# sloisel/MultiGridBarrier.jl

Measured on AMD Instinct MI355X. Metric: Newton iters/sec + wall-clock to converge, 2D P2 p-Laplace L=9, higher is better.
Workload: dtype f64

## Files before the change

multigridbarrier.jl_amd/csrc/driver.cpp:

```cpp
#include <chrono>
#include <cstdio>
#include <cstdlib>
#include <cmath>
#include <cstring>
#include <functional>
#include <limits>

#include "problem.hpp"

using namespace mgbhip;

namespace {

constexpr double EPS = std::numeric_limits<double>::epsilon();

bool debug_on() {
    static const bool on = env_on("MGBHIP_DEBUG");
    return on;
}
#define DBG(...) do { if (debug_on()) { fprintf(stderr, __VA_ARGS__); } } while (0)

struct Stop {
    double lambda_tol;
    double theta;
    int (*fn)(double, double, double, double, double, double, void*) = nullptr;
    void* user = nullptr;
    bool operator()(double ymin, double ynext, double gmin, double gnorm_next, double ndecmin, double ndec) const {
        if (fn) return fn(ymin, ynext, gmin, gnorm_next, ndecmin, ndec, user) != 0;
        const bool exact = (ynext >= ymin) && (gnorm_next >= theta * gmin);
        if (lambda_tol >= 0) return (ndec < lambda_tol) || exact;
        return exact;
    }
};

struct NewtonResult {
    int k = 0;
    bool converged = false;
    double y = 0;
};

struct VecStats { double sumsq, bad; };

VecStats vec_stats(mgbhip_problem* P, int level, const double* d_v, int64_t len) {
    hipStream_t st = P->stream();
    launch_vec_stats(d_v, len, P->d_scratch.p, P->d_scal.p + 2, st, P->own_mask(level));
    P->read_scalars(2, 2);
    if (P->sharded()) P->allreduce_host(P->pin.d + 2, 2, 0);
    return VecStats{P->pin.d[2], P->pin.d[3]};
}

double dev_dot(mgbhip_problem* P, int level, const double* a, const double* b, int64_t len) {
    hipStream_t st = P->stream();
    launch_dot(a, b, len, P->d_scratch.p, P->d_scal.p + 4, st, P->own_mask(level));
    P->read_scalars(4, 1);
    if (P->sharded()) P->allreduce_host(P->pin.d + 4, 1, 0);
    return P->pin.d[4];
}

struct NewtonCtx {
    mgbhip_problem* P;
    int level;
    const double* d_zJ;
    const double* d_c;
    int64_t m;
    double F0(const double* d_s) { return P->eval_f0(level, d_s, d_zJ, d_c); }
    void F1(const double* d_s, double* d_out, double* d_part) { P->eval_f1(level, d_s, d_zJ, d_c, d_out, P->sharded() ? d_part : nullptr); }
    const double* rhs_of_g() const { return P->sharded() ? P->d_gpart.p : P->d_g.p; }
    void F2(const double* d_s) { P->eval_f2(level, d_s, d_zJ, d_c, false, rhs_of_g()); }
};

bool trial_values(NewtonCtx& C, double& ynext, double& gnorm_next, int32_t* moved = nullptr, const double* step = nullptr,
                  bool* restrict_fused_out = nullptr) {
    mgbhip_problem* P = C.P;
    hipStream_t st = P->stream();
    const bool onfly = step && P->can_fuse_step(C.level);
    if (step) {
        ++P->step_stamp;
        if (!onfly) launch_step(P->d_x.p, P->d_nv.p, *step, P->d_xn.p, C.m, P->d_flag.p, P->step_stamp, st);
        P->touch();
    }
    const bool fused = !P->dense;
    static const bool fuse_restrict = !env_on("MGBHIP_NO_FUSED_RESTRICT");
    TrialRestrict fuse;
    TrialPoint point{};
    if (onfly) {
        point = TrialPoint{P->d_x.p, P->d_nv.p, *step};
        fuse = TrialRestrict{P->d_x.p, P->d_nv.p, *step, P->d_xn.p, P->d_flag.p, P->step_stamp};
    }
    const bool restrict_fused = P->eval_f01_launch(C.level, P->d_xn.p, C.d_zJ, C.d_c, P->d_gn.p, P->sharded() ? P->d_gnpart.p : nullptr, fused,
                                                   onfly ? &point : nullptr, (fused && fuse_restrict) ? &fuse : nullptr);
    if (restrict_fused_out) *restrict_fused_out = restrict_fused;
    if (onfly && !restrict_fused) launch_step(P->d_x.p, P->d_nv.p, *step, P->d_xn.p, C.m, P->d_flag.p, P->step_stamp, st);
    const double seq = P->next_seq();
    launch_trial_finish(P->d_gn.p, C.m, P->d_scratch.p, fused ? P->d_partials.p : nullptr, elem_grid(P->p, P->N), P->d_scal.p,
                        P->d_flag.p, P->pin.dev, st, P->own_mask(C.level), seq, restrict_fused);
    P->wait_results(seq);
    P->pin.i[0] = P->pin.d[4] == (double)P->step_stamp ? 1 : 0;
    if (P->sharded()) {
        P->pin.d[1] = (double)P->pin.i[0];
        P->allreduce_host(P->pin.d, 4, 0);
        P->pin.i[0] = P->pin.d[1] != 0.0 ? 1 : 0;
    }
    if (moved) *moved = P->pin.i[0];
    ynext = P->pin.d[0];
    if (!std::isfinite(ynext)) return false;
    if (P->pin.d[3] != 0.0 || !std::isfinite(P->pin.d[2])) return false;
    gnorm_next = std::sqrt(P->pin.d[2]);
    return true;
}

bool linesearch_backtracking(NewtonCtx& C, const mgbhip_options& opt, double y, double inc, double& ynext,
                             double& gnorm_next) {
    mgbhip_problem* P = C.P;
    hipStream_t st = P->stream();
    double s = 1.0;
    bool have = false;
    while (s > 0.0) {
        double yn, gn;
        int32_t moved = 0;
        if (trial_values(C, yn, gn, &moved, &s)) {
            have = true;
            ynext = yn;
            gnorm_next = gn;
            const bool stalled = (moved == 0);
            if (stalled || yn <= y - opt.ls_c1 * inc * s) return true;
        }
        s *= opt.ls_beta;
    }
    return have;
}

bool linesearch_illinois(NewtonCtx& C, const mgbhip_options& opt, double inc, double& ynext, double& gnorm_next) {
    mgbhip_problem* P = C.P;
    hipStream_t st = P->stream();
    struct Reject {};
    auto phi = [&](double sigma) -> double {
        launch_step(P->d_x.p, P->d_nv.p, sigma, P->d_xn.p, C.m, P->d_flag.p, ++P->step_stamp, st);
        P->touch();
        const double f = C.F0(P->d_xn.p);
        if (!std::isfinite(f)) throw Reject();
        C.F1(P->d_xn.p, P->d_gn.p, P->d_gnpart.p);
        const double v = dev_dot(P, C.level, P->d_gn.p, P->d_nv.p, C.m);
        if (!std::isfinite(v)) throw Reject();
        return v;
    };
    double s = 1.0;
    bool have = false;
    while (s > 0.0) {
        try {
            double a = 0.0, b = s, fa = inc, fb = phi(s), root = b;
            bool done = false;
            if (fa == 0) { root = a; done = true; }
            else if (fa * fb >= 0) { root = b; done = true; }
            for (int it = 0; it < 10000 && !done; ++it) {
                const double c = (a * fb - b * fa) / (fb - fa);
                const double fc = phi(c);
                if (c <= std::fmin(a, b) || c >= std::fmax(a, b) || fc * fa == 0 || fc * fb == 0) { root = c; done = true; break; }
                if (fb * fc < 0) { a = b; fa = fb; } else { fa /= 2; }
                b = c; fb = fc;
            }
            if (!done) throw Reject();
            launch_step(P->d_x.p, P->d_nv.p, root, P->d_xn.p, C.m, P->d_flag.p, ++P->step_stamp, st);
        P->touch();
            double yn, gn;
            if (!trial_values(C, yn, gn)) throw Reject();
            ynext = yn;
            gnorm_next = gn;
            return true;
        } catch (Reject&) {
        }
        s *= opt.ls_beta;
    }
    return have;
}

NewtonResult newton(NewtonCtx& C, const mgbhip_options& opt, const Stop& stop, int maxit) {
    mgbhip_problem* P = C.P;
    hipStream_t st = P->stream();
    NewtonResult R;
    P->d_x.zero(st, (size_t)C.m);
    P->touch();
    double y = C.F0(P->d_x.p);
    if (!std::isfinite(y)) throw InvalidArgument("newton: initial objective value is not finite");
    double ymin = y;
    if (P->sharded()) { P->d_gpart.ensure((size_t)C.m); P->d_gnpart.ensure((size_t)C.m); }
    C.F1(P->d_x.p, P->d_g.p, P->d_gpart.p);
    VecStats gs = vec_stats(P, C.level, P->d_g.p, C.m);
    if (gs.bad != 0.0 || !std::isfinite(gs.sumsq)) throw InvalidArgument("newton: initial gradient has non-finite entries");
    double gnorm = std::sqrt(gs.sumsq);
    double gmin = gnorm;
    double incmin = INFINITY;
    int k = 0;
    bool converged = false;
    Level& L = P->levels[C.level];
    struct RobustReset {
        MfSolver& s;
        ~RobustReset() { s.robust = false; }
    } robust_reset{L.solver};
    while (k < maxit && !converged) {
        ++k;
        C.F2(P->d_x.p);
        auto t0 = std::chrono::steady_clock::now();
        int fstatus = MGBHIP_OK;
        int leaf_flag = 0;
        for (int attempt = 0; attempt < 2; ++attempt) {
            P->factor(C.level, C.rhs_of_g());
            P->trisolve_carried(C.level, P->d_nv.p);
            const double seq = P->next_seq();
            launch_dir_finish(P->d_nv.p, P->d_g.p, C.m, P->d_scratch.p, P->d_scal.p, L.solver.status_flags_rw(), P->pin.dev, st,
                              P->own_mask(C.level), seq);
            L.solver.flags_cleared();
            P->wait_results(seq);
            P->pin.i[1] = P->pin.d[5] != 0.0 ? 1 : 0;
            leaf_flag |= P->pin.d[6] != 0.0 ? 1 : 0;
            P->pin.i[2] = leaf_flag;
            fstatus = MfSolver::status_from(P->pin.i + 1, L.solver.factored_condensed);
            if (P->sharded()) {
                P->pin.d[5] = fstatus != MGBHIP_OK ? 1.0 : 0.0;
                P->allreduce_host(P->pin.d + 2, 4, 0);
                fstatus = P->pin.d[5] != 0.0 ? MGBHIP_ERR_NOT_SPD : MGBHIP_OK;
            }
            const bool at_floor = std::fabs(P->pin.d[4]) <= EPS * std::fmax(std::fabs(y), 1.0);
            const bool suspicious = fstatus != MGBHIP_OK || P->pin.d[3] != 0.0 || !std::isfinite(P->pin.d[2]) ||
                                    (!(P->pin.d[4] > 0) && !at_floor);
            if (!suspicious || attempt == 1 || !L.solver.has_inverse_path() || L.solver.robust) break;
            DBG("newton[lev %d] k=%d: direction rejected (status %d, lambda^2=%.3e): refactoring with the substitution kernels\n",
                C.level, k, fstatus, P->pin.d[4]);
            L.solver.robust = true;
            L.H.drop_factors();
        }
        if (fstatus != MGBHIP_OK && P->lu_fallback(C.level, P->d_g.p, P->d_nv.p)) {
            DBG("newton[lev %d] k=%d: LDL' met a zero pivot; direction from the pivoted LU fallback\n", C.level, k);
            launch_dir_finish(P->d_nv.p, P->d_g.p, C.m, P->d_scratch.p, P->d_scal.p, L.solver.status_flags_rw(), P->pin.dev, st,
                              P->own_mask(C.level));
            L.solver.flags_cleared();
            MGB_HIP_CHECK(hipStreamSynchronize(st));
            fstatus = MGBHIP_OK;
        }
        P->cnt.solve_seconds += std::chrono::duration<double>(std::chrono::steady_clock::now() - t0).count();
        if (fstatus != MGBHIP_OK) {
            DBG("newton[lev %d] k=%d: Cholesky met a non-positive pivot (y=%.17g |g|=%.6e)\n", C.level, k, y, gnorm);
            converged = false;
            break;
        }
        if (P->pin.d[3] != 0.0 || !std::isfinite(P->pin.d[2])) throw InvalidArgument("newton: Newton direction has non-finite entries");
        const double inc = P->pin.d[4];
        DBG("newton[lev %d] k=%d y=%.17g |g|=%.6e lambda^2=%.6e\n", C.level, k, y, gnorm, inc);
        if (inc <= 0) {
            converged = std::fabs(inc) <= EPS * std::fmax(std::fabs(y), 1.0);
            break;
        }
        double ynext = y, gnorm_next = gnorm;
        bool moved = (opt.line_search == 1) ? linesearch_illinois(C, opt, inc, ynext, gnorm_next)
                                            : linesearch_backtracking(C, opt, y, inc, ynext, gnorm_next);
        if (!moved) {
            ynext = y;
            gnorm_next = gnorm;
        }
        if (stop(ymin, ynext, gmin, gnorm_next, std::sqrt(incmin), std::sqrt(inc))) converged = true;
        if (moved) {
            std::swap(P->d_x, P->d_xn);
            std::swap(P->d_g, P->d_gn);
            std::swap(P->d_gpart, P->d_gnpart);
        }
        y = ynext;
        gnorm = gnorm_next;
        gmin = std::fmin(gmin, gnorm);
        ymin = std::fmin(ymin, y);
        incmin = std::fmin(inc, incmin);
    }
    DBG("newton[lev %d] done k=%d converged=%d y=%.17g\n", C.level, k, (int)converged, y);
    R.k = k;
    R.converged = converged;
    R.y = y;
    P->cnt.newton += k;
    return R;
}

struct StepResult {
    bool converged;
    std::vector<int64_t> its;
};

StepResult mgb_step(mgbhip_problem* P, const double* d_c, const mgbhip_options& opt, bool finalize_now,
                    bool initial_step) {
    const int L = (int)P->levels.size();
    StepResult out;
    out.its.assign(L, 0);
    hipStream_t st = P->stream();
    const Stop sc{opt.stop_lambda_tol, opt.stop_theta, opt.stopping_criterion, opt.user};
    const Stop fin{-1.0, opt.finalize_theta};
    const size_t zn = (size_t)P->nu * P->n;
    auto eta = [&](int j, int J, const Stop& stop, int maxit) -> bool {
        (void)j;
        const int lev = J - 1;
        MGB_HIP_CHECK(hipMemcpyAsync(P->d_z0.p, P->d_z.p, zn * sizeof(double), hipMemcpyDeviceToDevice, st));
        NewtonCtx C{P, lev, P->d_z0.p, d_c, P->levels[lev].m};
        NewtonResult r = newton(C, opt, stop, maxit);
        out.its[lev] += r.k;
        if (r.converged) {
            const Level& Lv = P->levels[lev];
            StageScope scp(P->ctx->timers, "prolong");
            launch_csr_matvec(Lv.rows, Lv.Rptr.p, Lv.Rcol.p, Lv.Rval.p, P->d_x.p, P->d_z.p, true, false, st);
        }
        return r.converged;
    };
    std::function<bool(int, int)> dac = [&](int j, int J) -> bool {
        const int mn = (initial_step && J - j == 1) ? opt.maxit : opt.max_newton;
        if (eta(j, J, sc, mn)) return true;
        const int jmid = (j + J) / 2;
        if (jmid == j || jmid == J) return false;
        return dac(j, jmid) && dac(jmid, J);
    };
    bool converged = dac(0, L);
    if (finalize_now) {
        const bool foo = eta(L - 1, L, fin, opt.maxit);
        converged = converged && foo;
    }
    out.converged = converged;
    return out;
}

double c_dot_Dz(mgbhip_problem* P, const double* d_c) {
    hipStream_t st = P->stream();
    ElemParams E = P->elem_params(d_c);
    E.z0 = P->d_z.p;
    E.invn = 0.0;
    E.bw = nullptr;
    launch_elem(E, MODE_F0, st);
    launch_reduce_partials(P->d_partials.p, elem_grid(P->p, P->N), P->d_scal.p, st);
    double v;
    P->d_scal.download(&v, 1, st);
    MGB_HIP_CHECK(hipStreamSynchronize(st));
    if (P->sharded()) P->allreduce_host(&v, 1, 0);
    return v;
}

bool slack_feasible(mgbhip_problem* P, std::vector<double>& hbuf) {
    hipStream_t st = P->stream();
    hbuf.resize((size_t)P->n);
    MGB_HIP_CHECK(hipMemcpyAsync(hbuf.data(), P->d_z.p + (size_t)(P->nu - 1) * P->n, (size_t)P->n * sizeof(double),
                                 hipMemcpyDeviceToHost, st));
    MGB_HIP_CHECK(hipStreamSynchronize(st));
    double mx = -INFINITY;
    for (double v : hbuf) mx = std::fmax(mx, v);
    if (P->sharded()) P->allreduce_host(&mx, 1, 1);
    return mx < 0;
}

}

void trial_values_run(mgbhip_problem* P, int level, double step, double* y, int32_t* moved, int32_t* finite, int32_t* path) {
    NewtonCtx C{P, level, P->d_z0.p, P->d_c.p, P->levels[level].m};
    double yn = 0.0, gn = 0.0;
    const bool onfly = P->can_fuse_step(level);
    bool restrict_fused = false;
    *finite = trial_values(C, yn, gn, moved, &step, &restrict_fused) ? 1 : 0;
    *y = yn;
    *path = (onfly ? 1 : 0) | (restrict_fused ? 2 : 0);
}

int core_run(mgbhip_problem* P, double* z, const double* c, const mgbhip_options* optp, mgbhip_core_result* res) {
    const mgbhip_options opt = *optp;
    hipStream_t st = P->stream();
    const size_t zn = (size_t)P->nu * P->n;
    const size_t cn = (size_t)P->n * P->nD;
    const int L = (int)P->levels.size();
    P->prepare_all();
    P->d_z.upload(z, zn, st);
    P->d_c0.upload(c, cn, st);
    P->cnt = Counters();
    auto tb = std::chrono::steady_clock::now();
    auto now = [&] { return std::chrono::duration<double>(std::chrono::steady_clock::now() - tb).count(); };
    double t = opt.t;
    const double target = 1.0 / opt.tol;
    double kappa = opt.kappa;
    const double kappa0 = kappa;
    int k = 1;
    std::vector<double> hbuf;
    double t_first = INFINITY;
    std::vector<double> zhost;
    auto early = [&](double tt) -> bool {
        if (opt.early_stop_fn) {
            zhost.resize(zn);
            P->d_z.download(zhost.data(), zn, st);
            MGB_HIP_CHECK(hipStreamSynchronize(st));
            if (opt.early_stop_fn(zhost.data(), tt, opt.user) != 0) return true;
        }
        if (opt.early_stop != 1) return false;
        if (!slack_feasible(P, hbuf)) return false;
        t_first = std::fmin(t_first, tt);
        return tt >= 2 * t_first;
    };
    auto record = [&](int kk, const std::vector<int64_t>& its, bool add) {
        if (kk - 1 < res->cap_steps && res->its) {
            for (int l = 0; l < L; ++l) {
                if (add) res->its[(size_t)(kk - 1) * L + l] += its[l];
                else res->its[(size_t)(kk - 1) * L + l] = its[l];
            }
        }
    };
    auto setc = [&](double tt) { launch_scale_copy(P->d_c0.p, tt, P->d_c.p, (int64_t)cn, st); };
    res->failure_code = 0;
    res->L = L;
    if (res->times && res->cap_steps > 0) res->times[0] = now();
    setc(t);
    StepResult S = mgb_step(P, P->d_c.p, opt, opt.finalize && t >= target, true);
    if (!S.converged) {
        res->failure_code = 1;
        res->k = 1;
        res->t_final = t;
        res->t_elapsed = now();
        return MGBHIP_ERR_CONVERGENCE;
    }
    record(1, S.its, false);
    auto diag = [&](int kk) {
        if (kk - 1 < res->cap_steps) {
            if (res->ts) res->ts[kk - 1] = t;
            if (res->kappas) res->kappas[kk - 1] = kappa;
            if (res->c_dot_Dz) res->c_dot_Dz[kk - 1] = c_dot_Dz(P, P->d_c0.p);
        }
    };
    diag(1);
    bool stopped_early = false;
    while (t < target && kappa > 1 && k < opt.maxit) {
        if (early(t)) { stopped_early = true; break; }
        ++k;
        if (k - 1 < res->cap_steps && res->its)
            for (int l = 0; l < L; ++l) res->its[(size_t)(k - 1) * L + l] = 0;
        if (res->times && k - 1 < res->cap_steps) res->times[k - 1] = now();
        while (kappa > 1) {
            const double t1 = kappa * t;
            setc(t1);
            P->d_tmp.ensure(zn);
            MGB_HIP_CHECK(hipMemcpyAsync(P->d_tmp.p, P->d_z.p, zn * sizeof(double), hipMemcpyDeviceToDevice, st));
            S = mgb_step(P, P->d_c.p, opt, opt.finalize && t1 >= target, false);
            record(k, S.its, true);
            if (S.converged) {
                int64_t mx = 0;
                for (int64_t v : S.its) mx = std::max(mx, v);
                if ((double)mx <= opt.max_newton * 0.5) kappa = std::fmin(kappa0, kappa * kappa);
                t = t1;
                break;
            }
            MGB_HIP_CHECK(hipMemcpyAsync(P->d_z.p, P->d_tmp.p, zn * sizeof(double), hipMemcpyDeviceToDevice, st));
            kappa = std::sqrt(kappa);
        }
        diag(k);
    }
    bool converged = (t >= target) || stopped_early || early(t);
    res->k = k;
    res->t_final = t;
    res->t_elapsed = now();
    res->solve_seconds = P->cnt.solve_seconds;
    res->newton_iterations = P->cnt.newton;
    res->f0_evals = P->cnt.f0;
    res->f1_evals = P->cnt.f1;
    res->f2_evals = P->cnt.f2;
    res->factorizations = P->cnt.factor;
    P->d_z.download(z, zn, st);
    MGB_HIP_CHECK(hipStreamSynchronize(st));
    if (!converged) {
        res->failure_code = (kappa <= 1) ? 1 : 2;
        return MGBHIP_ERR_CONVERGENCE;
    }
    return MGBHIP_OK;
}

int matched_t_run(mgbhip_problem* P, const double* z, const double* c, double t_default, double* t_out) {
    hipStream_t st = P->stream();
    const size_t zn = (size_t)P->nu * P->n;
    const size_t cn = (size_t)P->n * P->nD;
    const int lev = (int)P->levels.size() - 1;
    const int64_t m = P->levels[lev].m;
    P->d_z0.upload(z, zn, st);
    P->d_c0.upload(c, cn, st);
    P->d_c.zero(st, cn);
    P->d_x.zero(st, (size_t)m);
    P->touch();
    *t_out = t_default;
    const bool sh = P->sharded();
    if (sh) { P->d_gpart.ensure((size_t)m); P->d_gnpart.ensure((size_t)m); }
    P->eval_f1(lev, P->d_x.p, P->d_z0.p, P->d_c.p, P->d_g.p, sh ? P->d_gpart.p : nullptr);
    P->eval_f1(lev, P->d_x.p, P->d_z0.p, P->d_c0.p, P->d_gn.p, sh ? P->d_gnpart.p : nullptr);
    launch_axpy(-1.0, P->d_g.p, P->d_gn.p, m, st);
    if (sh) launch_axpy(-1.0, P->d_gpart.p, P->d_gnpart.p, m, st);
    P->eval_f2(lev, P->d_x.p, P->d_z0.p, P->d_c0.p);
    if (sh) {
        P->d_tmp.ensure((size_t)m + 1);
        P->factor(lev, P->d_gpart.p);
        P->trisolve_carried(lev, P->d_tmp.p);
        int bad = P->levels[lev].solver.status(st) != MGBHIP_OK;
        MGB_HIP_CHECK(hipMemcpyAsync(P->d_nv.p, P->d_tmp.p, sizeof(double) * (size_t)m, hipMemcpyDeviceToDevice, st));
        P->levels[lev].H.drop_factors();
        P->factor(lev, P->d_gnpart.p);
        P->trisolve_carried(lev, P->d_tmp.p);
        bad |= P->levels[lev].solver.status(st) != MGBHIP_OK;
        MGB_HIP_CHECK(hipMemcpyAsync(P->d_xn.p, P->d_tmp.p, sizeof(double) * (size_t)m, hipMemcpyDeviceToDevice, st));
        double fb = bad ? 1.0 : 0.0;
        P->allreduce_host(&fb, 1, 0);
        if (fb != 0.0) return MGBHIP_OK;
    } else {
        P->factor(lev);
        if (P->levels[lev].solver.status(st) != MGBHIP_OK) return MGBHIP_OK;
        P->trisolve(lev, P->d_g.p, P->d_nv.p);
        P->trisolve(lev, P->d_gn.p, P->d_xn.p);
    }
    const double d = dev_dot(P, lev, P->d_gn.p, P->d_xn.p, m);
    const double b = dev_dot(P, lev, P->d_g.p, P->d_xn.p, m) + dev_dot(P, lev, P->d_gn.p, P->d_nv.p, m);
    if (!(d > 0)) return MGBHIP_OK;
    const double tstar = -b / (2 * d);
    if (!(std::isfinite(tstar) && tstar > 0)) return MGBHIP_OK;
    *t_out = std::fmin(std::fmax(tstar, std::sqrt(EPS)), t_default);
    return MGBHIP_OK;
}
```

multigridbarrier.jl_amd/csrc/reduce_kernels.hpp:

```cpp
#pragma once
#include <hip/hip_runtime.h>

#include "dsum.hpp"
#include "kernels.hpp"

namespace mgbhip {

namespace {


__global__ __launch_bounds__(256) void reduce_partials_kernel(const double* __restrict__ partials, int64_t count,
                                                              double* __restrict__ out) {
    __shared__ double red[256];
    const int tid = threadIdx.x;
    double s = 0.0;
    for (int64_t i = tid; i < count; i += 256) s += partials[i];
    red[tid] = s;
    __syncthreads();
    for (int off = 128; off > 0; off >>= 1) {
        if (tid < off) red[tid] += red[tid + off];
        __syncthreads();
    }
    if (tid == 0) out[0] = red[0];
}

template <int MODE>
__global__ __launch_bounds__(256) void block_reduce_kernel(const double* __restrict__ a, const double* __restrict__ b,
                                                           int64_t n, double* __restrict__ partials,
                                                           const double* __restrict__ mask) {
    __shared__ double red[256];
    __shared__ double red2[256];
    const int tid = threadIdx.x;
    double s = 0.0, bad = 0.0;
    for (int64_t i = (int64_t)blockIdx.x * 256 + tid; i < n; i += (int64_t)gridDim.x * 256) {
        const double v = a[i];
        const double w = mask ? mask[i] : 1.0;
        if (MODE == 0) s += mask ? w * (v * b[i]) : v * b[i];
        else {
            s += mask ? w * (v * v) : v * v;
            bad += isfinite(v) ? 0.0 : 1.0;
        }
    }
    red[tid] = s;
    red2[tid] = bad;
    __syncthreads();
    for (int off = 128; off > 0; off >>= 1) {
        if (tid < off) { red[tid] += red[tid + off]; red2[tid] += red2[tid + off]; }
        __syncthreads();
    }
    if (tid == 0) {
        partials[blockIdx.x] = red[0];
        if (MODE == 1) partials[gridDim.x + blockIdx.x] = red2[0];
    }
}

__global__ __launch_bounds__(256) void restrict_trial_kernel(int64_t rows, const int32_t* __restrict__ ptr, const int32_t* __restrict__ col,
                                                             const double* __restrict__ val, const double* __restrict__ ret,
                                                             double* __restrict__ g, double* __restrict__ partials,
                                                             const double* __restrict__ x, const double* __restrict__ nn, double s,
                                                             double* __restrict__ xn, int32_t* __restrict__ moved, int32_t stamp) {
    __shared__ double red[256];
    __shared__ double red2[256];
    __shared__ int any_moved;
    const int tid = threadIdx.x;
    if (tid == 0) any_moved = 0;
    __syncthreads();
    double ss = 0.0, bad = 0.0;
    bool m = false;
    for (int64_t i = (int64_t)blockIdx.x * 256 + tid; i < rows; i += (int64_t)gridDim.x * 256) {
        double acc = 0.0;
        for (int32_t q = ptr[i]; q < ptr[i + 1]; ++q) acc += val[q] * ret[col[q]];
        g[i] = acc;
        ss += acc * acc;
        bad += isfinite(acc) ? 0.0 : 1.0;
        if (xn) {
            const double xi = x[i];
            const double v = __builtin_fma(-s, nn[i], xi);
            xn[i] = v;
            m = m || (v != xi);
        }
    }
    red[tid] = ss;
    red2[tid] = bad;
    if (m) any_moved = 1;
    __syncthreads();
    for (int off = 128; off > 0; off >>= 1) {
        if (tid < off) { red[tid] += red[tid + off]; red2[tid] += red2[tid + off]; }
        __syncthreads();
    }
    if (tid == 0) {
        partials[blockIdx.x] = red[0];
        partials[gridDim.x + blockIdx.x] = red2[0];
        if (any_moved) *moved = stamp;
    }
}

__global__ __launch_bounds__(256) void dir_stats_kernel(const double* __restrict__ v, const double* __restrict__ g, int64_t n,
                                                        double* __restrict__ partials, const double* __restrict__ mask) {
    __shared__ double red[3][256];
    const int tid = threadIdx.x;
    double s = 0.0, bad = 0.0, d = 0.0;
    for (int64_t i = (int64_t)blockIdx.x * 256 + tid; i < n; i += (int64_t)gridDim.x * 256) {
        const double x = v[i];
        const double w = mask ? mask[i] : 1.0;
        s += mask ? w * (x * x) : x * x;
        bad += isfinite(x) ? 0.0 : 1.0;
        d += mask ? w * (g[i] * x) : g[i] * x;
    }
    red[0][tid] = s; red[1][tid] = bad; red[2][tid] = d;
    __syncthreads();
    for (int off = 128; off > 0; off >>= 1) {
        if (tid < off) {
            red[0][tid] += red[0][tid + off];
            red[1][tid] += red[1][tid + off];
            red[2][tid] += red[2][tid + off];
        }
        __syncthreads();
    }
    if (tid == 0) {
        partials[blockIdx.x] = red[0][0];
        partials[gridDim.x + blockIdx.x] = red[1][0];
        partials[2 * gridDim.x + blockIdx.x] = red[2][0];
    }
}

struct FinishJob { const double* src; int64_t count; int32_t out; };
struct FinishParams {
    FinishJob job[4];
    int32_t njobs;
    double* out;
    int32_t* ints;
    int32_t nints, ints_out, reset;
    double* host;
    int32_t host_lo, host_n;
    double seq;
};
__global__ __launch_bounds__(256) void finish_kernel(const FinishParams P) {
    __shared__ double red[256];
    __shared__ double res[16];
    const int tid = threadIdx.x;
    if (tid < P.nints) {
        res[P.ints_out + tid] = (double)P.ints[tid];
        if (P.reset) P.ints[tid] = 0;
    }
    for (int o = 0; o < P.njobs; ++o) {
        const double* __restrict__ src = P.job[o].src;
        const int64_t cnt = P.job[o].count;
        double s = 0.0;
        for (int64_t i = tid; i < cnt; i += 256) s += src[i];
        red[tid] = s;
        __syncthreads();
        for (int off = 128; off > 0; off >>= 1) {
            if (tid < off) red[tid] += red[tid + off];
            __syncthreads();
        }
        if (tid == 0) res[P.job[o].out] = red[0];
        __syncthreads();
    }
    __syncthreads();
    if (tid < 16) {
        bool mine = false;
        for (int o = 0; o < P.njobs; ++o) mine = mine || (P.job[o].out == tid);
        if (tid >= P.ints_out && tid < P.ints_out + P.nints) mine = true;
        if (mine) P.out[tid] = res[tid];
        if (P.host && tid >= P.host_lo && tid < P.host_lo + P.host_n) P.host[tid] = mine ? res[tid] : P.out[tid];
    }
    if (P.host && P.seq != 0.0) {
        __threadfence_system();
        __syncthreads();
        if (tid == 0) {
            __hip_atomic_store(P.host + 15, P.seq, __ATOMIC_RELEASE, __HIP_MEMORY_SCOPE_SYSTEM);
        }
    }
}

}

void launch_reduce_partials(const double* partials, int64_t count, double* out, hipStream_t st) {
    hipLaunchKernelGGL(reduce_partials_kernel, dim3(1), dim3(256), 0, st, partials, count, out);
    MGB_HIP_CHECK(hipGetLastError());
}

static int reduce_blocks(int64_t n);

int64_t reduce_scratch_doubles(int64_t n) { return 3 * (int64_t)reduce_blocks(n); }

static void launch_finish(const FinishParams& F, hipStream_t st) {
    hipLaunchKernelGGL(finish_kernel, dim3(1), dim3(256), 0, st, F);
    MGB_HIP_CHECK(hipGetLastError());
}

void launch_vec_stats(const double* v, int64_t n, double* scratch, double* stats, hipStream_t st, const double* mask,
                      const int32_t* ints, int nints) {
    const int nb = reduce_blocks(n);
    hipLaunchKernelGGL(block_reduce_kernel<1>, dim3(nb), dim3(256), 0, st, v, (const double*)nullptr, n, scratch, mask);
    FinishParams F{};
    F.job[0] = FinishJob{scratch, nb, 0};
    F.job[1] = FinishJob{scratch + nb, nb, 1};
    F.njobs = 2;
    F.out = stats;
    F.ints = const_cast<int32_t*>(ints); F.nints = nints; F.ints_out = 2; F.reset = 0;
    launch_finish(F, st);
}

void launch_dir_stats(const double* v, const double* g, int64_t n, double* scratch, double* stats3, hipStream_t st,
                      const double* mask, const int32_t* ints, int nints) {
    const int nb = reduce_blocks(n);
    hipLaunchKernelGGL(dir_stats_kernel, dim3(nb), dim3(256), 0, st, v, g, n, scratch, mask);
    FinishParams F{};
    F.job[0] = FinishJob{scratch, nb, 0};
    F.job[1] = FinishJob{scratch + nb, nb, 1};
    F.job[2] = FinishJob{scratch + 2 * nb, nb, 2};
    F.njobs = 3;
    F.out = stats3;
    F.ints = const_cast<int32_t*>(ints); F.nints = nints; F.ints_out = 3; F.reset = 0;
    launch_finish(F, st);
}

__global__ void publish_kernel(const double* __restrict__ src, int n, double* __restrict__ host, double* __restrict__ stamp, double seq) {
    const int tid = threadIdx.x;
    if (tid < n) host[tid] = src[tid];
    __threadfence_system();
    __syncthreads();
    if (tid == 0) __hip_atomic_store(stamp, seq, __ATOMIC_RELEASE, __HIP_MEMORY_SCOPE_SYSTEM);
}

void launch_publish(const double* src, int n, double* host_block, int host_lo, double seq, hipStream_t st) {
    hipLaunchKernelGGL(publish_kernel, dim3(1), dim3(64), 0, st, src, n, host_block + host_lo, host_block + 15, seq);
    MGB_HIP_CHECK(hipGetLastError());
}

void launch_dir_finish(const double* v, const double* g, int64_t n, double* scratch, double* scal, int32_t* status2, double* host,
                       hipStream_t st, const double* mask, double seq) {
    const int nb = reduce_blocks(n);
    hipLaunchKernelGGL(dir_stats_kernel, dim3(nb), dim3(256), 0, st, v, g, n, scratch, mask);
    FinishParams F{};
    F.job[0] = FinishJob{scratch, nb, 2};
    F.job[1] = FinishJob{scratch + nb, nb, 3};
    F.job[2] = FinishJob{scratch + 2 * nb, nb, 4};
    F.njobs = 3;
    F.out = scal;
    F.ints = status2; F.nints = 2; F.ints_out = 5; F.reset = 1;
    F.host = host; F.host_lo = 2; F.host_n = 5;
    F.seq = seq;
    launch_finish(F, st);
}

void launch_trial_finish(const double* g, int64_t n, double* scratch, const double* f0_partials, int64_t f0_count, double* scal,
                         int32_t* moved, double* host, hipStream_t st, const double* mask, double seq, bool partials_ready) {
    const int nb = reduce_blocks(n);
    if (!partials_ready) hipLaunchKernelGGL(block_reduce_kernel<1>, dim3(nb), dim3(256), 0, st, g, (const double*)nullptr, n, scratch, mask);
    FinishParams F{};
    int nj = 0;
    if (f0_partials) F.job[nj++] = FinishJob{f0_partials, f0_count, 0};
    F.job[nj++] = FinishJob{scratch, nb, 2};
    F.job[nj++] = FinishJob{scratch + nb, nb, 3};
    F.njobs = nj;
    F.out = scal;
    F.ints = moved; F.nints = 1; F.ints_out = 4; F.reset = 0;
    F.host = host; F.host_lo = 0; F.host_n = 5;
    F.seq = seq;
    launch_finish(F, st);
}

void launch_dot(const double* a, const double* b, int64_t n, double* scratch, double* out, hipStream_t st, const double* mask) {
    const int nb = reduce_blocks(n);
    hipLaunchKernelGGL(block_reduce_kernel<0>, dim3(nb), dim3(256), 0, st, a, b, n, scratch, mask);
    FinishParams F{};
    F.job[0] = FinishJob{scratch, nb, 0};
    F.njobs = 1;
    F.out = out;
    launch_finish(F, st);
}

void launch_restrict_trial(int64_t rows, const int32_t* ptr, const int32_t* col, const double* val, const double* ret, double* g,
                            double* scratch, const double* x, const double* nn, double s, double* xn, int32_t* moved, int32_t stamp,
                            hipStream_t st) {
    if (rows == 0) return;
    const int nb = reduce_blocks(rows);
    hipLaunchKernelGGL(restrict_trial_kernel, dim3(nb), dim3(256), 0, st, rows, ptr, col, val, ret, g, scratch, x, nn, s, xn, moved, stamp);
    MGB_HIP_CHECK(hipGetLastError());
}

}
```

Measured before the change: 691.5.

## Fuse Newton start evaluation, drop z snapshot copy, batch finish-kernel loads

```diff
diff --git a/multigridbarrier.jl_amd/csrc/driver.cpp b/multigridbarrier.jl_amd/csrc/driver.cpp
--- a/multigridbarrier.jl_amd/csrc/driver.cpp
+++ b/multigridbarrier.jl_amd/csrc/driver.cpp
@@ -180,12 +180,26 @@
     NewtonResult R;
     P->d_x.zero(st, (size_t)C.m);
     P->touch();
-    double y = C.F0(P->d_x.p);
-    if (!std::isfinite(y)) throw InvalidArgument("newton: initial objective value is not finite");
+    static const bool split_start = env_on("MGBHIP_SPLIT_START");
+    double y;
+    VecStats gs;
+    if (!split_start && !P->dense && !P->sharded() && opt.line_search != 1) {
+        P->eval_f01_launch(C.level, P->d_x.p, C.d_zJ, C.d_c, P->d_g.p, nullptr, true);
+        const double seq = P->next_seq();
+        launch_trial_finish(P->d_g.p, C.m, P->d_scratch.p, P->d_partials.p, elem_grid(P->p, P->N), P->d_scal.p, P->d_flag.p,
+                            P->pin.dev, st, P->own_mask(C.level), seq);
+        P->wait_results(seq);
+        y = P->pin.d[0];
+        if (!std::isfinite(y)) throw InvalidArgument("newton: initial objective value is not finite");
+        gs = VecStats{P->pin.d[2], P->pin.d[3]};
+    } else {
+        y = C.F0(P->d_x.p);
+        if (!std::isfinite(y)) throw InvalidArgument("newton: initial objective value is not finite");
+        if (P->sharded()) { P->d_gpart.ensure((size_t)C.m); P->d_gnpart.ensure((size_t)C.m); }
+        C.F1(P->d_x.p, P->d_g.p, P->d_gpart.p);
+        gs = vec_stats(P, C.level, P->d_g.p, C.m);
+    }
     double ymin = y;
-    if (P->sharded()) { P->d_gpart.ensure((size_t)C.m); P->d_gnpart.ensure((size_t)C.m); }
-    C.F1(P->d_x.p, P->d_g.p, P->d_gpart.p);
-    VecStats gs = vec_stats(P, C.level, P->d_g.p, C.m);
     if (gs.bad != 0.0 || !std::isfinite(gs.sumsq)) throw InvalidArgument("newton: initial gradient has non-finite entries");
     double gnorm = std::sqrt(gs.sumsq);
     double gmin = gnorm;
@@ -294,8 +308,9 @@
     auto eta = [&](int j, int J, const Stop& stop, int maxit) -> bool {
         (void)j;
         const int lev = J - 1;
-        MGB_HIP_CHECK(hipMemcpyAsync(P->d_z0.p, P->d_z.p, zn * sizeof(double), hipMemcpyDeviceToDevice, st));
-        NewtonCtx C{P, lev, P->d_z0.p, d_c, P->levels[lev].m};
+        static const bool snapshot = env_on("MGBHIP_Z_SNAPSHOT");
+        if (snapshot) MGB_HIP_CHECK(hipMemcpyAsync(P->d_z0.p, P->d_z.p, zn * sizeof(double), hipMemcpyDeviceToDevice, st));
+        NewtonCtx C{P, lev, snapshot ? P->d_z0.p : P->d_z.p, d_c, P->levels[lev].m};
         NewtonResult r = newton(C, opt, stop, maxit);
         out.its[lev] += r.k;
         if (r.converged) {
diff --git a/multigridbarrier.jl_amd/csrc/reduce_kernels.hpp b/multigridbarrier.jl_amd/csrc/reduce_kernels.hpp
--- a/multigridbarrier.jl_amd/csrc/reduce_kernels.hpp
+++ b/multigridbarrier.jl_amd/csrc/reduce_kernels.hpp
@@ -135,7 +135,81 @@
     int32_t host_lo, host_n;
     double seq;
 };
+constexpr int FINISH_LOADS_IN_FLIGHT = 8;
+template <int U>
 __global__ __launch_bounds__(256) void finish_kernel(const FinishParams P) {
+    __shared__ double red[4][256];
+    __shared__ double res[16];
+    const int tid = threadIdx.x;
+    if (tid < P.nints) {
+        res[P.ints_out + tid] = (double)P.ints[tid];
+        if (P.reset) P.ints[tid] = 0;
+    }
+    int64_t cnt[4], cmax = 0;
+#pragma unroll
+    for (int o = 0; o < 4; ++o) {
+        cnt[o] = o < P.njobs ? P.job[o].count : 0;
+        cmax = cnt[o] > cmax ? cnt[o] : cmax;
+    }
+    double s[4] = {0.0, 0.0, 0.0, 0.0};
+    for (int64_t base = 0; base < cmax; base += 256 * U) {
+        double v[4][U];
+#pragma unroll
+        for (int o = 0; o < 4; ++o) {
+            const double* __restrict__ src = P.job[o].src;
+            if (base < cnt[o]) {
+#pragma unroll
+                for (int u = 0; u < U; ++u) {
+                    const int64_t i = base + u * 256 + tid;
+                    v[o][u] = src[i < cnt[o] ? i : cnt[o] - 1];
+                }
+            } else {
+#pragma unroll
+                for (int u = 0; u < U; ++u) v[o][u] = 0.0;
+            }
+        }
+#pragma unroll
+        for (int o = 0; o < 4; ++o) {
+#pragma unroll
+            for (int u = 0; u < U; ++u) {
+                const int64_t i = base + u * 256 + tid;
+                if (i < cnt[o]) s[o] += v[o][u];
+            }
+        }
+    }
+#pragma unroll
+    for (int o = 0; o < 4; ++o) red[o][tid] = s[o];
+    __syncthreads();
+    for (int off = 128; off > 0; off >>= 1) {
+        if (tid < off) {
+#pragma unroll
+            for (int o = 0; o < 4; ++o) red[o][tid] += red[o][tid + off];
+        }
+        __syncthreads();
+    }
+    if (tid == 0) {
+#pragma unroll
+        for (int o = 0; o < 4; ++o)
+            if (o < P.njobs) res[P.job[o].out] = red[o][0];
+    }
+    __syncthreads();
+    if (tid < 16) {
+        bool mine = false;
+        for (int o = 0; o < P.njobs; ++o) mine = mine || (P.job[o].out == tid);
+        if (tid >= P.ints_out && tid < P.ints_out + P.nints) mine = true;
+        if (mine) P.out[tid] = res[tid];
+        if (P.host && tid >= P.host_lo && tid < P.host_lo + P.host_n) P.host[tid] = mine ? res[tid] : P.out[tid];
+    }
+    if (P.host && P.seq != 0.0) {
+        __threadfence_system();
+        __syncthreads();
+        if (tid == 0) {
+            __hip_atomic_store(P.host + 15, P.seq, __ATOMIC_RELEASE, __HIP_MEMORY_SCOPE_SYSTEM);
+        }
+    }
+}
+
+__global__ __launch_bounds__(256) void finish_serial_kernel(const FinishParams P) {
     __shared__ double red[256];
     __shared__ double res[16];
     const int tid = threadIdx.x;
@@ -186,7 +260,9 @@
 int64_t reduce_scratch_doubles(int64_t n) { return 3 * (int64_t)reduce_blocks(n); }
 
 static void launch_finish(const FinishParams& F, hipStream_t st) {
-    hipLaunchKernelGGL(finish_kernel, dim3(1), dim3(256), 0, st, F);
+    static const bool serial = env_on("MGBHIP_FINISH_SERIAL");
+    if (serial) hipLaunchKernelGGL(finish_serial_kernel, dim3(1), dim3(256), 0, st, F);
+    else hipLaunchKernelGGL(finish_kernel<FINISH_LOADS_IN_FLIGHT>, dim3(1), dim3(256), 0, st, F);
     MGB_HIP_CHECK(hipGetLastError());
 }
 
```

After: 700.2 (median of 6 runs). 1.01x the previous value.
